# igormq/aes-lac-2018

Measured on AMD Instinct MI355X. Metric: train frames/sec, DeepSpeech2 5xBiGRU-800, higher is better.
Workload: dtype f32

## Files before the change

### aes-lac-2018_amd/csrc/bn.hip

```cpp
#include "ds2_common.h"

namespace {

constexpr int NPART = 64;

template <int MODE>
__global__ __launch_bounds__(256) void bn2d_reduce_kernel(const float* __restrict__ x, const float* __restrict__ dy,
                                                          const float* __restrict__ mean_invstd,
                                                          const float* __restrict__ gamma,
                                                          const float* __restrict__ beta, int B, int C, int inner,
                                                          double* __restrict__ part) {
    const int c = blockIdx.y, p = blockIdx.x, tid = threadIdx.x;
    const int chunks = (inner + 1023) / 1024;
    const int items = B * chunks;
    float mu = 0.f, is = 0.f, ga = 0.f, be = 0.f;
    if (MODE == 1) {
        mu = mean_invstd[c];
        is = mean_invstd[C + c];
        ga = gamma[c];
        be = beta[c];
    }
    float s0 = 0.f, s1 = 0.f;
    for (int it = p; it < items; it += NPART) {
        const int b = it / chunks, ch = it % chunks;
        const size_t base = ((size_t)b * C + c) * inner;
        const int i0 = ch * 1024;
#pragma unroll
        for (int u = 0; u < 4; ++u) {
            const int i = i0 + u * 256 + tid;
            if (i < inner) {
                const float v = x[base + i];
                if (MODE == 0) {
                    s0 += v;
                    s1 += v * v;
                } else {
                    const float xh = (v - mu) * is;
                    const float y = ga * xh + be;
                    const float g = (y > 0.f && y < 20.f) ? dy[base + i] : 0.f;
                    s0 += g;
                    s1 += g * xh;
                }
            }
        }
    }
    double d0 = wave_sum_d((double)s0), d1 = wave_sum_d((double)s1);
    __shared__ double sm[4][2];
    if ((tid & 63) == 0) {
        sm[tid >> 6][0] = d0;
        sm[tid >> 6][1] = d1;
    }
    __syncthreads();
    if (tid == 0) {
        part[((size_t)c * NPART + p) * 2 + 0] = sm[0][0] + sm[1][0] + sm[2][0] + sm[3][0];
        part[((size_t)c * NPART + p) * 2 + 1] = sm[0][1] + sm[1][1] + sm[2][1] + sm[3][1];
    }
}

template <int MODE>
__global__ __launch_bounds__(256) void bn2d_reduce_vec_kernel(const float* __restrict__ x, const float* __restrict__ dy,
                                                              const float* __restrict__ mean_invstd,
                                                              const float* __restrict__ gamma,
                                                              const float* __restrict__ beta, int B, int C, int inner,
                                                              double* __restrict__ part) {
    const int c = blockIdx.y, p = blockIdx.x, tid = threadIdx.x;
    const int chunks = (inner + 1023) / 1024;
    const int items = B * chunks;
    float mu = 0.f, is = 0.f, ga = 0.f, be = 0.f;
    if (MODE == 1) {
        mu = mean_invstd[c];
        is = mean_invstd[C + c];
        ga = gamma[c];
        be = beta[c];
    }
    float s0 = 0.f, s1 = 0.f;
    auto take = [&](float v, float g) {
        if (MODE == 0) {
            s0 += v;
            s1 += v * v;
        } else {
            const float xh = (v - mu) * is;
            const float y = ga * xh + be;
            const float gm = (y > 0.f && y < 20.f) ? g : 0.f;
            s0 += gm;
            s1 += gm * xh;
        }
    };
    for (int it = p; it < items; it += NPART) {
        const int b = it / chunks, ch = it % chunks;
        const size_t base = ((size_t)b * C + c) * inner;
        const int h = min((int)((4 - (base & 3)) & 3), inner);
        const int nq = (inner - h) >> 2;
        const int q = ch * 256 + tid;
        if (q < nq) {
            const f32x4 v = *reinterpret_cast<const f32x4*>(x + base + h + 4 * (size_t)q);
            f32x4 g = {0.f, 0.f, 0.f, 0.f};
            if (MODE == 1) g = *reinterpret_cast<const f32x4*>(dy + base + h + 4 * (size_t)q);
#pragma unroll
            for (int e = 0; e < 4; ++e) take(v[e], g[e]);
        }
        if (ch == 0) {
            const int tail0 = h + 4 * nq, e = tid < 4 ? tid : tail0 + tid - 4;
            if ((tid < h) || (tid >= 4 && tid < 8 && e < inner)) take(x[base + e], MODE == 1 ? dy[base + e] : 0.f);
        }
    }
    double d0 = wave_sum_d((double)s0), d1 = wave_sum_d((double)s1);
    __shared__ double sm[4][2];
    if ((tid & 63) == 0) {
        sm[tid >> 6][0] = d0;
        sm[tid >> 6][1] = d1;
    }
    __syncthreads();
    if (tid == 0) {
        part[((size_t)c * NPART + p) * 2 + 0] = sm[0][0] + sm[1][0] + sm[2][0] + sm[3][0];
        part[((size_t)c * NPART + p) * 2 + 1] = sm[0][1] + sm[1][1] + sm[2][1] + sm[3][1];
    }
}

template <int MODE>
__global__ __launch_bounds__(256) void bn1d_reduce_kernel(const float* __restrict__ xa, const float* __restrict__ xb,
                                                          const float* __restrict__ dy,
                                                          const float* __restrict__ mean_invstd, int rows, int F,
                                                          double* __restrict__ part) {
    const int p = blockIdx.x, tid = threadIdx.x;
    const int col = blockIdx.y * 64 + (tid & 63), ry = tid >> 6;
    float mu = 0.f, is = 0.f;
    if (MODE == 1 && col < F) {
        mu = mean_invstd[col];
        is = mean_invstd[F + col];
    }
    float s0 = 0.f, s1 = 0.f;
    if (col < F) {
        for (int r = p * 4 + ry; r < rows; r += NPART * 4) {
            const size_t o = (size_t)r * F + col;
            float v = xa[o];
            if (xb) v += xb[o];
            if (MODE == 0) {
                s0 += v;
                s1 += v * v;
            } else {
                const float g = dy[o];
                s0 += g;
                s1 += g * (v - mu) * is;
            }
        }
    }
    __shared__ float sm[4][64][2];
    sm[ry][tid & 63][0] = s0;
    sm[ry][tid & 63][1] = s1;
    __syncthreads();
    if (ry == 0 && col < F) {
        const int l = tid & 63;
        const double d0 = (double)sm[0][l][0] + (double)sm[1][l][0] + (double)sm[2][l][0] + (double)sm[3][l][0];
        const double d1 = (double)sm[0][l][1] + (double)sm[1][l][1] + (double)sm[2][l][1] + (double)sm[3][l][1];
        part[((size_t)col * NPART + p) * 2 + 0] = d0;
        part[((size_t)col * NPART + p) * 2 + 1] = d1;
    }
}

__global__ __launch_bounds__(64) void bn_finalize_stats_kernel(const double* __restrict__ part, int C, double count,
                                                               float eps, float momentum, int use_running,
                                                               float* __restrict__ running_mean,
                                                               float* __restrict__ running_var,
                                                               float* __restrict__ mean_invstd) {
    const int c = blockIdx.x, lane = threadIdx.x;
    if (use_running) {
        if (lane == 0) {
            mean_invstd[c] = running_mean[c];
            mean_invstd[C + c] = (float)(1.0 / sqrt((double)running_var[c] + (double)eps));
        }
        return;
    }
    double s0 = part[((size_t)c * NPART + lane) * 2 + 0];
    double s1 = part[((size_t)c * NPART + lane) * 2 + 1];
    s0 = wave_sum_d(s0);
    s1 = wave_sum_d(s1);
    if (lane == 0) {
        const double mean = s0 / count;
        double var = s1 / count - mean * mean;
        if (var < 0.0) var = 0.0;
        mean_invstd[c] = (float)mean;
        mean_invstd[C + c] = (float)(1.0 / sqrt(var + (double)eps));
        if (running_mean) {
            const double unb = count > 1.0 ? var * count / (count - 1.0) : var;
            running_mean[c] = (float)((1.0 - momentum) * running_mean[c] + momentum * mean);
            running_var[c] = (float)((1.0 - momentum) * running_var[c] + momentum * unb);
        }
    }
}

__global__ __launch_bounds__(64) void bn_finalize_bwd_kernel(const double* __restrict__ part, int C, double count,
                                                             float* __restrict__ dgamma, float* __restrict__ dbeta,
                                                             float* __restrict__ coef) {
    const int c = blockIdx.x, lane = threadIdx.x;
    double s0 = part[((size_t)c * NPART + lane) * 2 + 0];
    double s1 = part[((size_t)c * NPART + lane) * 2 + 1];
    s0 = wave_sum_d(s0);
    s1 = wave_sum_d(s1);
    if (lane == 0) {
        dbeta[c] = (float)s0;
        dgamma[c] = (float)s1;
        coef[c] = (float)(s0 / count);
        coef[C + c] = (float)(s1 / count);
    }
}

__global__ __launch_bounds__(256) void bn2d_apply_kernel(const float* __restrict__ x,
                                                         const float* __restrict__ mean_invstd,
                                                         const float* __restrict__ gamma,
                                                         const float* __restrict__ beta, int C, int inner,
                                                         float* __restrict__ y) {
    const int bc = blockIdx.y, c = bc % C;
    const float sc = gamma[c] * mean_invstd[C + c];
    const float sh = beta[c] - mean_invstd[c] * sc;
    const size_t base = (size_t)bc * inner;
    for (int i = blockIdx.x * 256 + threadIdx.x; i < inner; i += gridDim.x * 256) {
        const float v = x[base + i] * sc + sh;
        y[base + i] = fminf(fmaxf(v, 0.f), 20.f);
    }
}

__global__ __launch_bounds__(256) void bn2d_apply_tbf_kernel(const float* __restrict__ x,
                                                             const float* __restrict__ mean_invstd,
                                                             const float* __restrict__ gamma,
                                                             const float* __restrict__ beta, int B, int C, int D,
                                                             int T, float* __restrict__ y) {
    __shared__ float tile[32][33];
    const int b = blockIdx.z;
    const int CD = C * D;
    const int t0 = blockIdx.x * 32, f0 = blockIdx.y * 32;
    const int tx = threadIdx.x & 31, ty = threadIdx.x >> 5;
#pragma unroll
    for (int i = 0; i < 32; i += 8) {
        const int f = f0 + ty + i, t = t0 + tx;
        if (f < CD && t < T) {
            const int c = f / D;
            const float sc = gamma[c] * mean_invstd[C + c];
            const float sh = beta[c] - mean_invstd[c] * sc;
            const float v = x[((size_t)b * CD + f) * T + t] * sc + sh;
            tile[ty + i][tx] = fminf(fmaxf(v, 0.f), 20.f);
        }
    }
    __syncthreads();
#pragma unroll
    for (int i = 0; i < 32; i += 8) {
        const int t = t0 + ty + i, f = f0 + tx;
        if (f < CD && t < T) y[((size_t)t * B + b) * CD + f] = tile[tx][ty + i];
    }
}

__global__ __launch_bounds__(256) void bn2d_bwd_apply_kernel(const float* __restrict__ x, const float* __restrict__ dy,
                                                             const float* __restrict__ mean_invstd,
                                                             const float* __restrict__ gamma,
                                                             const float* __restrict__ beta,
                                                             const float* __restrict__ coef, int C, int inner,
                                                             float* __restrict__ dx) {
    const int bc = blockIdx.y, c = bc % C;
    const float mu = mean_invstd[c], is = mean_invstd[C + c], ga = gamma[c], be = beta[c];
    const float mg = coef[c], mgx = coef[C + c];
    const size_t base = (size_t)bc * inner;
    for (int i = blockIdx.x * 256 + threadIdx.x; i < inner; i += gridDim.x * 256) {
        const float xh = (x[base + i] - mu) * is;
        const float yv = ga * xh + be;
        const float g = (yv > 0.f && yv < 20.f) ? dy[base + i] : 0.f;
        dx[base + i] = ga * is * (g - mg - xh * mgx);
    }
}

template <typename F>
__device__ __forceinline__ void bn2d_row_vec(size_t base, int inner, F&& f4, int bx, int nbx, int tid) {
    const int h = min((int)((4 - (base & 3)) & 3), inner);
    const int nq = (inner - h) >> 2;
    for (int q = bx * 256 + tid; q < nq; q += nbx * 256) f4(base + h + 4 * (size_t)q, 4);
    if (bx == 0) {
        const int tail0 = h + 4 * nq, e = tid < 4 ? tid : tail0 + tid - 4;
        if ((tid < h) || (tid >= 4 && tid < 8 && e < inner)) f4(base + e, 1);
    }
}

__global__ __launch_bounds__(256) void bn2d_bwd_apply_vec_kernel(const float* __restrict__ x, const float* __restrict__ dy,
                                                                 const float* __restrict__ mean_invstd,
                                                                 const float* __restrict__ gamma,
                                                                 const float* __restrict__ beta,
                                                                 const float* __restrict__ coef, int C, int inner,
                                                                 float* __restrict__ dx) {
    const int bc = blockIdx.y, c = bc % C;
    const float mu = mean_invstd[c], is = mean_invstd[C + c], ga = gamma[c], be = beta[c];
    const float mg = coef[c], mgx = coef[C + c];
    auto one = [&](float xv, float g) {
        const float xh = (xv - mu) * is;
        const float yv = ga * xh + be;
        const float gm = (yv > 0.f && yv < 20.f) ? g : 0.f;
        return ga * is * (gm - mg - xh * mgx);
    };
    bn2d_row_vec((size_t)bc * inner, inner, [&](size_t o, int n) {
        if (n == 4) {
            const f32x4 xv = *reinterpret_cast<const f32x4*>(x + o), g = *reinterpret_cast<const f32x4*>(dy + o);
            f32x4 r;
#pragma unroll
            for (int e = 0; e < 4; ++e) r[e] = one(xv[e], g[e]);
            *reinterpret_cast<f32x4*>(dx + o) = r;
        } else {
            dx[o] = one(x[o], dy[o]);
        }
    }, blockIdx.x, gridDim.x, threadIdx.x);
}

__global__ __launch_bounds__(256) void bn2d_apply_vec_kernel(const float* __restrict__ x,
                                                             const float* __restrict__ mean_invstd,
                                                             const float* __restrict__ gamma,
                                                             const float* __restrict__ beta, int C, int inner,
                                                             float* __restrict__ y) {
    const int bc = blockIdx.y, c = bc % C;
    const float sc = gamma[c] * mean_invstd[C + c];
    const float sh = beta[c] - mean_invstd[c] * sc;
    bn2d_row_vec((size_t)bc * inner, inner, [&](size_t o, int n) {
        if (n == 4) {
            const f32x4 xv = *reinterpret_cast<const f32x4*>(x + o);
            f32x4 r;
#pragma unroll
            for (int e = 0; e < 4; ++e) r[e] = fminf(fmaxf(xv[e] * sc + sh, 0.f), 20.f);
            *reinterpret_cast<f32x4*>(y + o) = r;
        } else {
            y[o] = fminf(fmaxf(x[o] * sc + sh, 0.f), 20.f);
        }
    }, blockIdx.x, gridDim.x, threadIdx.x);
}

__global__ __launch_bounds__(256) void bn1d_apply_kernel(const float* __restrict__ xa, const float* __restrict__ xb,
                                                         const float* __restrict__ mean_invstd,
                                                         const float* __restrict__ gamma,
                                                         const float* __restrict__ beta, size_t n, int F,
                                                         float* __restrict__ y) {
    const size_t stride = (size_t)gridDim.x * 256;
    for (size_t i = (size_t)blockIdx.x * 256 + threadIdx.x; i < n; i += stride) {
        const int col = (int)(i % F);
        float v = xa[i];
        if (xb) v += xb[i];
        const float sc = gamma[col] * mean_invstd[F + col];
        y[i] = (v - mean_invstd[col]) * sc + beta[col];
    }
}

__global__ __launch_bounds__(256) void bn1d_bwd_apply_kernel(const float* __restrict__ xa, const float* __restrict__ xb,
                                                             const float* __restrict__ dy,
                                                             const float* __restrict__ mean_invstd,
                                                             const float* __restrict__ gamma,
                                                             const float* __restrict__ coef, size_t n, int F,
                                                             float* __restrict__ dx) {
    const size_t stride = (size_t)gridDim.x * 256;
    for (size_t i = (size_t)blockIdx.x * 256 + threadIdx.x; i < n; i += stride) {
        const int col = (int)(i % F);
        float v = xa[i];
        if (xb) v += xb[i];
        const float is = mean_invstd[F + col];
        const float xh = (v - mean_invstd[col]) * is;
        dx[i] = gamma[col] * is * (dy[i] - coef[col] - xh * coef[F + col]);
    }
}

template <int MODE>
__global__ __launch_bounds__(256) void bn1d_reduce_vec_kernel(const f32x4* __restrict__ xa, const f32x4* __restrict__ xb,
                                                              const f32x4* __restrict__ dy,
                                                              const float* __restrict__ mean_invstd, int rows, int F,
                                                              double* __restrict__ part) {
    const int p = blockIdx.x, tid = threadIdx.x;
    const int F4 = F >> 2;
    const int cq = blockIdx.y * 64 + (tid & 63), ry = tid >> 6;
    f32x4 mu = {0.f, 0.f, 0.f, 0.f}, is = mu;
    if (MODE == 1 && cq < F4) {
        mu = *reinterpret_cast<const f32x4*>(mean_invstd + 4 * cq);
        is = *reinterpret_cast<const f32x4*>(mean_invstd + F + 4 * cq);
    }
    f32x4 s0 = {0.f, 0.f, 0.f, 0.f}, s1 = s0;
    if (cq < F4) {
        for (int r = p * 4 + ry; r < rows; r += NPART * 4) {
            const size_t o = (size_t)r * F4 + cq;
            f32x4 v = xa[o];
            if (xb) v += xb[o];
            if (MODE == 0) {
                s0 += v;
                s1 += v * v;
            } else {
                const f32x4 g = dy[o];
                s0 += g;
                s1 += g * (v - mu) * is;
            }
        }
    }
    __shared__ f32x4 sm[4][64][2];
    sm[ry][tid & 63][0] = s0;
    sm[ry][tid & 63][1] = s1;
    __syncthreads();
    if (ry == 0 && cq < F4) {
        const int l = tid & 63;
#pragma unroll
        for (int e = 0; e < 4; ++e) {
            const double d0 = (double)sm[0][l][0][e] + (double)sm[1][l][0][e] + (double)sm[2][l][0][e] + (double)sm[3][l][0][e];
            const double d1 = (double)sm[0][l][1][e] + (double)sm[1][l][1][e] + (double)sm[2][l][1][e] + (double)sm[3][l][1][e];
            part[((size_t)(4 * cq + e) * NPART + p) * 2 + 0] = d0;
            part[((size_t)(4 * cq + e) * NPART + p) * 2 + 1] = d1;
        }
    }
}

__global__ __launch_bounds__(256) void bn1d_apply_vec_kernel(const f32x4* __restrict__ xa, const f32x4* __restrict__ xb,
                                                             const float* __restrict__ mean_invstd,
                                                             const float* __restrict__ gamma,
                                                             const float* __restrict__ beta, size_t n4, int F4,
                                                             f32x4* __restrict__ y) {
    const size_t stride = (size_t)gridDim.x * 256;
    for (size_t i = (size_t)blockIdx.x * 256 + threadIdx.x; i < n4; i += stride) {
        const int c = 4 * (int)(i % F4);
        f32x4 v = xa[i];
        if (xb) v += xb[i];
        const f32x4 sc = *reinterpret_cast<const f32x4*>(gamma + c) * *reinterpret_cast<const f32x4*>(mean_invstd + 4 * F4 + c);
        y[i] = (v - *reinterpret_cast<const f32x4*>(mean_invstd + c)) * sc + *reinterpret_cast<const f32x4*>(beta + c);
    }
}

__global__ __launch_bounds__(256) void bn1d_bwd_apply_vec_kernel(const f32x4* __restrict__ xa, const f32x4* __restrict__ xb,
                                                                 const f32x4* __restrict__ dy,
                                                                 const float* __restrict__ mean_invstd,
                                                                 const float* __restrict__ gamma,
                                                                 const float* __restrict__ coef, size_t n4, int F4,
                                                                 f32x4* __restrict__ dx) {
    const size_t stride = (size_t)gridDim.x * 256;
    const int F = 4 * F4;
    for (size_t i = (size_t)blockIdx.x * 256 + threadIdx.x; i < n4; i += stride) {
        const int c = 4 * (int)(i % F4);
        f32x4 v = xa[i];
        if (xb) v += xb[i];
        const f32x4 is = *reinterpret_cast<const f32x4*>(mean_invstd + F + c);
        const f32x4 xh = (v - *reinterpret_cast<const f32x4*>(mean_invstd + c)) * is;
        dx[i] = *reinterpret_cast<const f32x4*>(gamma + c) * is *
                (dy[i] - *reinterpret_cast<const f32x4*>(coef + c) - xh * *reinterpret_cast<const f32x4*>(coef + F + c));
    }
}

inline bool aligned16(const void* p) { return ((uintptr_t)p & 15) == 0; }
inline bool vec4_ok(int F, const void* a, const void* b, const void* c, const void* d) {
    return (F & 3) == 0 && ((((uintptr_t)a) | ((uintptr_t)b) | ((uintptr_t)c) | ((uintptr_t)d)) & 15) == 0;
}

inline int ew_blocks(size_t n) {
    size_t b = (n + 255) / 256;
    if (b > 4096) b = 4096;
    if (b < 1) b = 1;
    return (int)b;
}

}

extern "C" size_t ds2_bn_ws_bytes(int C) { return (size_t)C * NPART * 2 * sizeof(double) + (size_t)C * 2 * sizeof(float); }

extern "C" int ds2_bn2d_stats(const float* x, int B, int C, int inner, float eps, float momentum, int use_running,
                              float* running_mean, float* running_var, float* mean_invstd, void* ws, void* stream) {
    DS2_CHECK_ARG(x && mean_invstd && ws && B > 0 && C > 0 && inner > 0);
    DS2_CHECK_ARG(!use_running || (running_mean && running_var));
    hipStream_t st = (hipStream_t)stream;
    double* part = (double*)ws;
    if (!use_running) {
        if (aligned16(x))
            hipLaunchKernelGGL((bn2d_reduce_vec_kernel<0>), dim3(NPART, C), dim3(256), 0, st, x, nullptr, nullptr, nullptr,
                               nullptr, B, C, inner, part);
        else
            hipLaunchKernelGGL((bn2d_reduce_kernel<0>), dim3(NPART, C), dim3(256), 0, st, x, nullptr, nullptr, nullptr,
                               nullptr, B, C, inner, part);
    }
    hipLaunchKernelGGL(bn_finalize_stats_kernel, dim3(C), dim3(64), 0, st, part, C, (double)B * inner, eps, momentum,
                       use_running, running_mean, running_var, mean_invstd);
    DS2_CHECK_LAUNCH();
    return DS2_OK;
}

extern "C" int ds2_bn2d_apply_htanh(const float* x, const float* mean_invstd, const float* gamma, const float* beta,
                                    int B, int C, int D, int T, int layout_tbf, float* y, void* stream) {
    DS2_CHECK_ARG(x && mean_invstd && gamma && beta && y && B > 0 && C > 0 && D > 0 && T > 0);
    hipStream_t st = (hipStream_t)stream;
    if (layout_tbf) {
        DS2_CHECK_ARG(B <= 65535);
        dim3 grid(ds2_cdiv(T, 32), ds2_cdiv(C * D, 32), B);
        hipLaunchKernelGGL(bn2d_apply_tbf_kernel, grid, dim3(256), 0, st, x, mean_invstd, gamma, beta, B, C, D, T, y);
    } else {
        const int inner = D * T;
        if (aligned16(x) && aligned16(y)) {
            dim3 grid(min(ds2_cdiv(inner, 1024), 64), B * C);
            hipLaunchKernelGGL(bn2d_apply_vec_kernel, grid, dim3(256), 0, st, x, mean_invstd, gamma, beta, C, inner, y);
        } else {
            dim3 grid(min(ds2_cdiv(inner, 256), 64), B * C);
            hipLaunchKernelGGL(bn2d_apply_kernel, grid, dim3(256), 0, st, x, mean_invstd, gamma, beta, C, inner, y);
        }
    }
    DS2_CHECK_LAUNCH();
    return DS2_OK;
}

extern "C" int ds2_bn2d_htanh_bwd(const float* x, const float* dy, const float* mean_invstd, const float* gamma,
                                  const float* beta, int B, int C, int D, int T, float* dx, float* dgamma,
                                  float* dbeta, void* ws, void* stream) {
    DS2_CHECK_ARG(x && dy && mean_invstd && gamma && beta && dx && dgamma && dbeta && ws);
    DS2_CHECK_ARG(B > 0 && C > 0 && D > 0 && T > 0);
    hipStream_t st = (hipStream_t)stream;
    const int inner = D * T;
    double* part = (double*)ws;
    float* coef = (float*)(part + (size_t)C * NPART * 2);
    const bool vec = aligned16(x) && aligned16(dy) && aligned16(dx);
    if (vec)
        hipLaunchKernelGGL((bn2d_reduce_vec_kernel<1>), dim3(NPART, C), dim3(256), 0, st, x, dy, mean_invstd, gamma, beta,
                           B, C, inner, part);
    else
        hipLaunchKernelGGL((bn2d_reduce_kernel<1>), dim3(NPART, C), dim3(256), 0, st, x, dy, mean_invstd, gamma, beta, B,
                           C, inner, part);
    hipLaunchKernelGGL(bn_finalize_bwd_kernel, dim3(C), dim3(64), 0, st, part, C, (double)B * inner, dgamma, dbeta,
                       coef);
    if (vec) {
        dim3 grid(min(ds2_cdiv(inner, 1024), 64), B * C);
        hipLaunchKernelGGL(bn2d_bwd_apply_vec_kernel, grid, dim3(256), 0, st, x, dy, mean_invstd, gamma, beta, coef, C,
                           inner, dx);
    } else {
        dim3 grid(min(ds2_cdiv(inner, 256), 64), B * C);
        hipLaunchKernelGGL(bn2d_bwd_apply_kernel, grid, dim3(256), 0, st, x, dy, mean_invstd, gamma, beta, coef, C, inner,
                           dx);
    }
    DS2_CHECK_LAUNCH();
    return DS2_OK;
}

extern "C" int ds2_bn1d_stats(const float* xa, const float* xb, int rows, int F, float eps, float momentum,
                              int use_running, float* running_mean, float* running_var, float* mean_invstd, void* ws,
                              void* stream) {
    DS2_CHECK_ARG(xa && mean_invstd && ws && rows > 0 && F > 0);
    DS2_CHECK_ARG(!use_running || (running_mean && running_var));
    hipStream_t st = (hipStream_t)stream;
    double* part = (double*)ws;
    if (!use_running) {
        if (vec4_ok(F, xa, xb, nullptr, nullptr))
            hipLaunchKernelGGL((bn1d_reduce_vec_kernel<0>), dim3(NPART, ds2_cdiv(F / 4, 64)), dim3(256), 0, st,
                               (const f32x4*)xa, (const f32x4*)xb, nullptr, nullptr, rows, F, part);
        else
            hipLaunchKernelGGL((bn1d_reduce_kernel<0>), dim3(NPART, ds2_cdiv(F, 64)), dim3(256), 0, st, xa, xb, nullptr,
                               nullptr, rows, F, part);
    }
    hipLaunchKernelGGL(bn_finalize_stats_kernel, dim3(F), dim3(64), 0, st, part, F, (double)rows, eps, momentum,
                       use_running, running_mean, running_var, mean_invstd);
    DS2_CHECK_LAUNCH();
    return DS2_OK;
}

extern "C" int ds2_bn1d_apply(const float* xa, const float* xb, const float* mean_invstd, const float* gamma,
                              const float* beta, int rows, int F, float* y, void* stream) {
    DS2_CHECK_ARG(xa && mean_invstd && gamma && beta && y && rows > 0 && F > 0);
    const size_t n = (size_t)rows * F;
    if (vec4_ok(F, xa, xb, y, gamma) && vec4_ok(F, beta, mean_invstd, nullptr, nullptr))
        hipLaunchKernelGGL(bn1d_apply_vec_kernel, dim3(ew_blocks(n / 4)), dim3(256), 0, (hipStream_t)stream,
                           (const f32x4*)xa, (const f32x4*)xb, mean_invstd, gamma, beta, n / 4, F / 4, (f32x4*)y);
    else
        hipLaunchKernelGGL(bn1d_apply_kernel, dim3(ew_blocks(n)), dim3(256), 0, (hipStream_t)stream, xa, xb,
                           mean_invstd, gamma, beta, n, F, y);
    DS2_CHECK_LAUNCH();
    return DS2_OK;
}

extern "C" int ds2_bn1d_bwd(const float* xa, const float* xb, const float* dy, const float* mean_invstd,
                            const float* gamma, int rows, int F, float* dx, float* dgamma, float* dbeta, void* ws,
                            void* stream) {
    DS2_CHECK_ARG(xa && dy && mean_invstd && gamma && dx && dgamma && dbeta && ws && rows > 0 && F > 0);
    hipStream_t st = (hipStream_t)stream;
    double* part = (double*)ws;
    float* coef = (float*)(part + (size_t)F * NPART * 2);
    const bool vec = vec4_ok(F, xa, xb, dy, dx) && vec4_ok(F, gamma, mean_invstd, nullptr, nullptr);
    if (vec)
        hipLaunchKernelGGL((bn1d_reduce_vec_kernel<1>), dim3(NPART, ds2_cdiv(F / 4, 64)), dim3(256), 0, st,
                           (const f32x4*)xa, (const f32x4*)xb, (const f32x4*)dy, mean_invstd, rows, F, part);
    else
        hipLaunchKernelGGL((bn1d_reduce_kernel<1>), dim3(NPART, ds2_cdiv(F, 64)), dim3(256), 0, st, xa, xb, dy,
                           mean_invstd, rows, F, part);
    hipLaunchKernelGGL(bn_finalize_bwd_kernel, dim3(F), dim3(64), 0, st, part, F, (double)rows, dgamma, dbeta, coef);
    const size_t n = (size_t)rows * F;
    if (vec)
        hipLaunchKernelGGL(bn1d_bwd_apply_vec_kernel, dim3(ew_blocks(n / 4)), dim3(256), 0, st, (const f32x4*)xa,
                           (const f32x4*)xb, (const f32x4*)dy, mean_invstd, gamma, coef, n / 4, F / 4, (f32x4*)dx);
    else
        hipLaunchKernelGGL(bn1d_bwd_apply_kernel, dim3(ew_blocks(n)), dim3(256), 0, st, xa, xb, dy, mean_invstd, gamma,
                           coef, n, F, dx);
    DS2_CHECK_LAUNCH();
    return DS2_OK;
}
```

### aes-lac-2018_amd/ds2hip/ops.py

```python
import os

import torch

from . import lib

F_BINS = 161
BN_EPS = 1e-5
BN_MOMENTUM = 0.1


def _empty(shape, like, dtype=torch.float32):
    return torch.empty(shape, dtype=dtype, device=like.device)


def _bytes_ws(nbytes, like):
    return torch.empty((int(nbytes) + 15) // 16 * 2, dtype=torch.float64, device=like.device)


def conv_out_frames(t_in):
    t1 = (t_in + 20 - 11) // 2 + 1
    return t1, t1 - 10


def spectrogram(wav, wav_offsets, t_max, normalize=True, eps=1e-9):
# ... 121 lines not shown
            ev.record()
            self.ring[host_tensor.dtype][i] = (buf, ev, False)
        return out

    def stage(self, host_tensor):
        n = host_tensor.numel()
        with self.lock:
            i, buf = self._slot(host_tensor.dtype, n, busy=True)
            view = buf[:n]
            view.copy_(host_tensor.reshape(-1))
        return i, view

    def staged_done(self, dtype, i):
        ev = torch.cuda.Event()
        ev.record()
        with self.lock:
            self.ring[dtype][i] = (self.ring[dtype][i][0], ev, False)

    def download(self, dev_tensor):
        n = dev_tensor.numel()
        with self.lock:
            i, buf = self._slot(dev_tensor.dtype, n)
            buf[:n].copy_(dev_tensor.reshape(-1), non_blocking=True)
            ev = torch.cuda.Event()
            ev.record()
            self.ring[dev_tensor.dtype][i] = (buf, ev, False)
        return buf[:n], ev


_pinned = _PinnedRing()
_staged = _PinnedRing()


def upload_small(host_tensor, device):
    return _pinned.upload(host_tensor, device)


def download_small(dev_tensor):
    return _pinned.download(dev_tensor)


def spin_wait(event):
    import time
    while not event.query():
        time.sleep(0)


def low_priority_stream(device):
    import ctypes
    with torch.cuda.device(device):
        out = ctypes.c_void_p()
        rc = lib.load().ds2_stream_create(1, ctypes.byref(out))
        if rc != 0:
            raise RuntimeError('ds2_stream_create failed (%d): %s' % (rc, lib.load().ds2_last_error().decode()))
        return torch.cuda.ExternalStream(out.value, device=device)

def gemm(a, b, trans_a=False, trans_b=False, out=None, beta=0.0, m=None, n=None, k=None, lda=None, ldb=None,
         ldc=None, split_k=1):
    if m is None:
        m = a.shape[1] if trans_a else a.shape[0]
    if k is None:
        k = a.shape[0] if trans_a else a.shape[1]
    if n is None:
        n = b.shape[0] if trans_b else b.shape[1]
    if lda is None:
        lda = a.shape[-1]
    if ldb is None:
        ldb = b.shape[-1]
    if out is None:
        out = _empty((m, n), a)
    if ldc is None:
        ldc = out.shape[-1]
    lib.call('ds2_gemm_f32', int(trans_a), int(trans_b), m, n, k, a, lda, b, ldb, out, ldc, float(beta), split_k)
    return out


def gemm_split_mode(mode=-1):
    return int(lib.load().ds2_gemm_split_mode(int(mode)))


def gemm_raw(trans_a, trans_b, m, n, k, a_ptr, lda, b_ptr, ldb, c_ptr, ldc, beta=0.0, split_k=1):
    lib.call('ds2_gemm_f32', int(trans_a), int(trans_b), m, n, k, a_ptr, lda, b_ptr, ldb, c_ptr, ldc, float(beta),
             split_k)


def gemm_tn_group(problems, n, k, accumulate=False):
    import ctypes
    cnt = len(problems)
    assert 1 <= cnt <= 4
    vp, ip = ctypes.c_void_p * cnt, ctypes.c_int * cnt
    a, lda, m, b, ldb, c, ldc = zip(*problems)
    args = (vp(*a), ip(*lda), ip(*m), vp(*b), ip(*ldb), vp(*c), ip(*ldc))
    fn = lib.load().ds2_gemm_f32_tn_group
    rc = fn(cnt, *[ctypes.cast(x, ctypes.c_void_p) for x in args], int(n), int(k), int(bool(accumulate)),
            lib.stream_ptr())
    if rc != 0:
        raise lib.Ds2Error(rc, 'ds2_gemm_f32_tn_group failed (%d): %s' % (rc, lib.load().ds2_last_error().decode()))


def transpose2d(x, rows, cols, out=None):
    if out is None:
        out = _empty((cols, rows), x)
    lib.call('ds2_transpose2d', x, rows, cols, out)
    return out


def transpose2d_group(tensors, batch, rows, cols, out):
    import ctypes
    cnt = len(tensors)
    assert 1 <= cnt <= 8 and all(t.is_cuda and t.is_contiguous() and t.numel() == batch * rows * cols for t in tensors)
    assert out.is_cuda and out.is_contiguous() and out.numel() == cnt * batch * rows * cols
    ptrs = (ctypes.c_void_p * cnt)(*[t.data_ptr() for t in tensors])
    rc = lib.load().ds2_transpose2d_group(cnt, ctypes.cast(ptrs, ctypes.c_void_p), int(batch), int(rows), int(cols),
                                          out.data_ptr(), lib.stream_ptr())
    if rc != 0:
        raise lib.Ds2Error(rc, 'ds2_transpose2d_group failed (%d): %s' % (rc, lib.load().ds2_last_error().decode()))
    return out


def add2(a, b):
    out = torch.empty_like(a)
    lib.call('ds2_add2', a, b, a.numel(), out)
    return out


def transpose_btf(x):
    bsz, t, f = x.shape
    out = _empty((bsz, f, t), x)
    lib.call('ds2_transpose_btf_to_bft', x, bsz, t, f, out)
    return out


def conv_fwd(which, inp, weight, bias, t_in):
    bsz = inp.shape[0]
    t1, t2 = conv_out_frames(t_in) if which == 1 else (None, t_in - 10)
    out = _empty((bsz, 32, 61, t1), inp) if which == 1 else _empty((bsz, 32, 21, t2), inp)
    ws = _empty((lib.query('ds2_conv_wt_ws_floats', which),), inp)
    lib.call('ds2_conv_fwd', which, inp, weight, bias, bsz, t_in, out, ws)
    return out


def conv2_dgrad(d_out, weight, t1):
    bsz = d_out.shape[0]
    d_in = _empty((bsz, 32, 61, t1), d_out)
    ws = _empty((lib.query('ds2_conv2_dgrad_ws_floats', bsz, t1),), d_out)
    lib.call('ds2_conv2_dgrad', d_out, weight, bsz, t1, d_in, ws, ws.numel())
    return d_in


def conv_wgrad(which, inp, d_out, t_in, d_weight, d_bias):
    lib.call('ds2_conv_wgrad', which, inp, d_out, inp.shape[0], t_in, d_weight, d_bias)


def _bn_ws(c, like):
    return _bytes_ws(lib.query('ds2_bn_ws_bytes', c), like)


def bn2d_stats(x, running_mean, running_var, training):
    bsz, c = x.shape[0], x.shape[1]
    inner = x.numel() // (bsz * c)
    mi = _empty((2 * c,), x)
    lib.call('ds2_bn2d_stats', x, bsz, c, inner, BN_EPS, BN_MOMENTUM, int(not training), running_mean, running_var, mi,
             _bn_ws(c, x))
    return mi


def bn2d_apply_htanh(x, mi, gamma, beta, layout_tbf):
    bsz, c, d, t = x.shape
    y = _empty((t, bsz, c * d), x) if layout_tbf else torch.empty_like(x)
    lib.call('ds2_bn2d_apply_htanh', x, mi, gamma, beta, bsz, c, d, t, int(layout_tbf), y)
    return y


def bn2d_htanh_bwd(x, dy, mi, gamma, beta, dgamma, dbeta):
    bsz, c, d, t = x.shape
    dx = torch.empty_like(x)
    lib.call('ds2_bn2d_htanh_bwd', x, dy, mi, gamma, beta, bsz, c, d, t, dx, dgamma, dbeta, _bn_ws(c, x))
    return dx


def bn1d_stats(xa, xb, rows, feat, running_mean, running_var, training):
    mi = _empty((2 * feat,), xa)
    lib.call('ds2_bn1d_stats', xa, xb, rows, feat, BN_EPS, BN_MOMENTUM, int(not training), running_mean, running_var,
             mi, _bn_ws(feat, xa))
    return mi


def bn1d_apply(xa, xb, mi, gamma, beta, rows, feat):
    y = _empty((rows, feat), xa)
    lib.call('ds2_bn1d_apply', xa, xb, mi, gamma, beta, rows, feat, y)
    return y


def bn1d_bwd(xa, xb, dy, mi, gamma, rows, feat, dgamma, dbeta):
    dx = _empty((rows, feat), xa)
    lib.call('ds2_bn1d_bwd', xa, xb, dy, mi, gamma, rows, feat, dx, dgamma, dbeta, _bn_ws(feat, xa))
    return dx


def _host_ints(vals):
    import ctypes
    return ctypes.cast((ctypes.c_int * len(vals))(*[int(v) for v in vals]), ctypes.c_void_p)


def _host_ptrs(tensors):
    import ctypes
    ptrs = []
    for t in tensors:
        if t is not None:
            assert t.is_cuda and t.is_contiguous()
        ptrs.append(None if t is None else t.data_ptr())
    return ctypes.cast((ctypes.c_void_p * len(ptrs))(*ptrs), ctypes.c_void_p)


def bn1d_seg_stats(xa, xb, t, bsz, feat, bounds, running_means, running_vars, training):
    g = len(bounds) - 1
    mi = _empty((g, 2 * feat), xa)
    lib.call('ds2_bn1d_seg_stats', xa, xb, t, bsz, feat, g, _host_ints(bounds), BN_EPS, BN_MOMENTUM, int(not training),
             _host_ptrs(running_means), _host_ptrs(running_vars), mi, _bytes_ws(g * lib.query('ds2_bn_ws_bytes', feat), xa))
    return mi


def bn1d_seg_apply(xa, xb, mi, t, bsz, feat, bounds, gammas, betas):
    y = _empty((t * bsz, feat), xa)
    lib.call('ds2_bn1d_seg_apply', xa, xb, mi, t, bsz, feat, len(bounds) - 1, _host_ints(bounds), _host_ptrs(gammas),
             _host_ptrs(betas), y)
    return y


def bn1d_seg_bwd(xa, xb, dxf, mi, t, bsz, feat, bounds, gammas, dgammas, dbetas):
    g = len(bounds) - 1
    dy = _empty((t * bsz, feat), xa)
    lib.call('ds2_bn1d_seg_bwd', xa, xb, dxf, mi, t, bsz, feat, g, _host_ints(bounds), _host_ptrs(gammas), dy,
             _host_ptrs(dgammas), _host_ptrs(dbetas), _bytes_ws(g * lib.query('ds2_bn_ws_bytes', feat), xa))
    return dy


GRU_MODE = os.environ.get('DS2_GRU_MODE', 'auto')
_sync_ws = {}
fallback_count = 0
_persistent_off = {}


def _dev_key(dev):
    return (dev.type, dev.index if dev.index is not None else torch.cuda.current_device())


def _gru_sync_ws(dev, bsz, hid):
    key = _dev_key(dev)
    n = (lib.query('ds2_gru_sync_ws_bytes', bsz, hid) + 3) // 4
    if key not in _sync_ws or _sync_ws[key].numel() < n:
        old = _sync_ws.get(key)
        if old is not None:
            word = lib.query('ds2_gru_sync_error_offset') // 4
            if int(old[word].item()) != 0:
                raise_async_error()
            _err_ptr_tables.clear()
        _sync_ws[key] = torch.zeros(n, dtype=torch.int32, device=dev)
    return _sync_ws[key]


def _use_persistent(dev, bsz, hid):
    if GRU_MODE == 'step':
        return False
    if _dev_key(dev) in _persistent_off:
        if GRU_MODE == 'persistent':
            raise RuntimeError('persistent GRU kernels are disabled on %s: %s' % (dev, _persistent_off[_dev_key(dev)]))
        return False
    ok = bool(lib.query('ds2_gru_persistent_supported', bsz, hid))
    if GRU_MODE == 'persistent' and not ok:
        raise RuntimeError('persistent GRU kernel does not support B=%d H=%d on this device' % (bsz, hid))
    return ok


def _disable_persistent(dev, reason):
    import logging
    global fallback_count
    fallback_count += 1
    if os.environ.get('DS2_GRU_STRICT', '0') == '1':
        raise RuntimeError('ds2hip: the persistent GRU kernels would fall back to the launch-per-step kernels on %s (%s) '
                           'and DS2_GRU_STRICT=1 forbids it' % (dev, reason))
    _persistent_off[_dev_key(dev)] = reason
    logging.getLogger('aes-lac-2018').warning('ds2hip: persistent GRU kernels disabled on %s (%s); using the '
                                              'launch-per-step kernels', dev, reason)


def async_error_words():
    word = lib.query('ds2_gru_sync_error_offset') // 4
    return [ws[word:word + 1] for ws in _sync_ws.values()]


def raise_async_error():
    for key, ws in _sync_ws.items():
        word = lib.query('ds2_gru_sync_error_offset') // 4
        bad = int(ws[word].item()) != 0
        ws.zero_()
        if bad:
            _disable_persistent(ws.device, 'a hand-off spin timed out (were all workgroups resident?)')
    raise RuntimeError('ds2hip: persistent GRU kernel timed out waiting for a workgroup hand-off; the results of this '
                       'step are invalid')


def check_async_errors():
    for w in async_error_words():
        if int(w.item()) != 0:
            raise_async_error()


_dh_supported = {}


def gru_bwd_dh_wanted(dev, bsz, hid):
    if not _use_persistent(dev, bsz, hid):
        return False
    key = (bsz, hid)
    if key not in _dh_supported:
        _dh_supported[key] = bool(lib.query('ds2_gru_bwd_dh_supported', bsz, hid))
    if not _dh_supported[key]:
        return False
    e = os.environ.get('DS2_GRU_BWD_DH')
    if e in ('0', '1'):
        return e == '1'
    return bsz >= 9


def gru_bidir_fwd(gates, w_hh, t, bsz, hid, want_coef=False):
    ghn = _empty((t, bsz, 2, hid), gates)
    hout = _empty((2, t, bsz, hid), gates)
    coef = _empty((t, bsz, 2, 3 * hid), gates) if want_coef and gru_bwd_dh_wanted(gates.device, bsz, hid) else None
    if _use_persistent(gates.device, bsz, hid):
        try:
            lib.call('ds2_gru_bidir_fwd_persistent_ex', gates, ghn, hout, w_hh, coef, _gru_sync_ws(gates.device, bsz, hid), t,
                     bsz, hid)
            return (ghn, hout, coef) if want_coef else (ghn, hout)
        except lib.Ds2Error as e:
            if e.code != lib.ERR_UNSUPPORTED or GRU_MODE == 'persistent':
                raise
            _disable_persistent(gates.device, str(e))
    lib.call('ds2_gru_bidir_fwd', gates, ghn, hout, w_hh, t, bsz, hid)
    return (ghn, hout, None) if want_coef else (ghn, hout)


def gru_bwd_coef(gates, ghn, hout, t, bsz, hid):
    coef = _empty((t, bsz, 2, 3 * hid), gates)
    lib.call('ds2_gru_bwd_coef', gates, ghn, hout, coef, t, bsz, hid)
    return coef


def gru_bidir_bwd(gates, ghn, hout, d_out, w_hh_t, t, bsz, hid, spare_cus=-1, coef=None):
# ... 144 lines not shown
```

Baseline: 565,000.

## Fuse BN finalize into reduce kernels via last-block atomic counter

Removes the separate BN finalize kernels. Each reduce kernel stores its partial sums with relaxed atomics, and the last block for each channel, found through an atomic counter, does the final sum and writes the stats or gradient coefficients. The partial layout changes to [p][k][C] to suit the in-kernel sum, and workspaces are cached and zero-initialised per device, stream and channel count so the counters start at zero. This saves one kernel launch per BN call. In exchange it adds atomic and ordering risk and shares cached workspaces between calls with the same channel count.

```diff
diff --git a/aes-lac-2018_amd/csrc/bn.hip b/aes-lac-2018_amd/csrc/bn.hip
--- a/aes-lac-2018_amd/csrc/bn.hip
+++ b/aes-lac-2018_amd/csrc/bn.hip
@@ -3,13 +3,100 @@
 namespace {
 
 constexpr int NPART = 64;
+
+struct BnFinal {
+    unsigned int* counter;
+    double count;
+    float eps, momentum;
+    float* running_mean;
+    float* running_var;
+    float* mi_out;
+    float* dgamma;
+    float* dbeta;
+    float* coef;
+};
+
+__device__ __forceinline__ size_t part_at(int p, int k, int C, int c) { return ((size_t)p * 2 + k) * C + c; }
+
+__device__ __forceinline__ void part_store(double* part, size_t i, double v) {
+    __hip_atomic_store(part + i, v, __ATOMIC_RELAXED, __HIP_MEMORY_SCOPE_AGENT);
+}
+__device__ __forceinline__ double part_load(const double* part, size_t i) {
+    return __hip_atomic_load(part + i, __ATOMIC_RELAXED, __HIP_MEMORY_SCOPE_AGENT);
+}
+
+__device__ __forceinline__ bool bn_last_block(unsigned int* counter, unsigned int total) {
+    __shared__ unsigned int last;
+    if (threadIdx.x < 64) {
+        __builtin_amdgcn_s_waitcnt(0x0F70);
+        asm volatile("" ::: "memory");
+        if (threadIdx.x == 0) {
+            last = atomicAdd(counter, 1u) == total - 1 ? 1u : 0u;
+            if (last) atomicExch(counter, 0u);
+        }
+    }
+    __syncthreads();
+    return last != 0u;
+}
+
+__device__ __forceinline__ double bn_tree_sum(const double* part, int C, int c, int k) {
+    double v[NPART];
+#pragma unroll
+    for (int p = 0; p < NPART; ++p) v[p] = part_load(part, part_at(p, k, C, c));
+#pragma unroll
+    for (int o = NPART / 2; o > 0; o >>= 1)
+#pragma unroll
+        for (int i = 0; i < o; ++i) v[i] += v[i + o];
+    return v[0];
+}
+
+template <int MODE>
+__device__ __forceinline__ void bn_finish(double s0, double s1, int c, int C, const BnFinal& f) {
+    if (MODE == 0) {
+        const double mean = s0 / f.count;
+        double var = s1 / f.count - mean * mean;
+        if (var < 0.0) var = 0.0;
+        f.mi_out[c] = (float)mean;
+        f.mi_out[C + c] = (float)(1.0 / sqrt(var + (double)f.eps));
+        if (f.running_mean) {
+            const double unb = f.count > 1.0 ? var * f.count / (f.count - 1.0) : var;
+            f.running_mean[c] = (float)((1.0 - f.momentum) * f.running_mean[c] + f.momentum * mean);
+            f.running_var[c] = (float)((1.0 - f.momentum) * f.running_var[c] + f.momentum * unb);
+        }
+    } else {
+        f.dbeta[c] = (float)s0;
+        f.dgamma[c] = (float)s1;
+        f.coef[c] = (float)(s0 / f.count);
+        f.coef[C + c] = (float)(s1 / f.count);
+    }
+}
+
+template <int MODE>
+__device__ __forceinline__ void bn2d_finalize(const double* part, int C, int c, const BnFinal& f) {
+    if (!bn_last_block(f.counter + c, NPART)) return;
+    const int lane = threadIdx.x;
+    if (lane >= 64) return;
+    const double s0 = wave_sum_d(part_load(part, part_at(lane, 0, C, c)));
+    const double s1 = wave_sum_d(part_load(part, part_at(lane, 1, C, c)));
+    if (lane == 0) bn_finish<MODE>(s0, s1, c, C, f);
+}
+
+template <int MODE>
+__device__ __forceinline__ void bn1d_finalize(const double* part, int F, int ncols, const BnFinal& f) {
+    if (!bn_last_block(f.counter + blockIdx.y, NPART)) return;
+    const int col = blockIdx.y * ncols + threadIdx.x;
+    if ((int)threadIdx.x >= ncols || col >= F) return;
+    const double s0 = bn_tree_sum(part, F, col, 0);
+    const double s1 = bn_tree_sum(part, F, col, 1);
+    bn_finish<MODE>(s0, s1, col, F, f);
+}
 
 template <int MODE>
 __global__ __launch_bounds__(256) void bn2d_reduce_kernel(const float* __restrict__ x, const float* __restrict__ dy,
                                                           const float* __restrict__ mean_invstd,
                                                           const float* __restrict__ gamma,
                                                           const float* __restrict__ beta, int B, int C, int inner,
-                                                          double* __restrict__ part) {
+                                                          double* part, BnFinal fin) {
     const int c = blockIdx.y, p = blockIdx.x, tid = threadIdx.x;
     const int chunks = (inner + 1023) / 1024;
     const int items = B * chunks;
@@ -51,9 +138,10 @@
     }
     __syncthreads();
     if (tid == 0) {
-        part[((size_t)c * NPART + p) * 2 + 0] = sm[0][0] + sm[1][0] + sm[2][0] + sm[3][0];
-        part[((size_t)c * NPART + p) * 2 + 1] = sm[0][1] + sm[1][1] + sm[2][1] + sm[3][1];
-    }
+        part_store(part, part_at(p, 0, C, c), sm[0][0] + sm[1][0] + sm[2][0] + sm[3][0]);
+        part_store(part, part_at(p, 1, C, c), sm[0][1] + sm[1][1] + sm[2][1] + sm[3][1]);
+    }
+    bn2d_finalize<MODE>(part, C, c, fin);
 }
 
 template <int MODE>
@@ -61,7 +149,7 @@
                                                               const float* __restrict__ mean_invstd,
                                                               const float* __restrict__ gamma,
                                                               const float* __restrict__ beta, int B, int C, int inner,
-                                                              double* __restrict__ part) {
+                                                              double* part, BnFinal fin) {
     const int c = blockIdx.y, p = blockIdx.x, tid = threadIdx.x;
     const int chunks = (inner + 1023) / 1024;
     const int items = B * chunks;
@@ -111,16 +199,17 @@
     }
     __syncthreads();
     if (tid == 0) {
-        part[((size_t)c * NPART + p) * 2 + 0] = sm[0][0] + sm[1][0] + sm[2][0] + sm[3][0];
-        part[((size_t)c * NPART + p) * 2 + 1] = sm[0][1] + sm[1][1] + sm[2][1] + sm[3][1];
-    }
+        part_store(part, part_at(p, 0, C, c), sm[0][0] + sm[1][0] + sm[2][0] + sm[3][0]);
+        part_store(part, part_at(p, 1, C, c), sm[0][1] + sm[1][1] + sm[2][1] + sm[3][1]);
+    }
+    bn2d_finalize<MODE>(part, C, c, fin);
 }
 
 template <int MODE>
 __global__ __launch_bounds__(256) void bn1d_reduce_kernel(const float* __restrict__ xa, const float* __restrict__ xb,
                                                           const float* __restrict__ dy,
                                                           const float* __restrict__ mean_invstd, int rows, int F,
-                                                          double* __restrict__ part) {
+                                                          double* part, BnFinal fin) {
     const int p = blockIdx.x, tid = threadIdx.x;
     const int col = blockIdx.y * 64 + (tid & 63), ry = tid >> 6;
     float mu = 0.f, is = 0.f;
@@ -152,55 +241,19 @@
         const int l = tid & 63;
         const double d0 = (double)sm[0][l][0] + (double)sm[1][l][0] + (double)sm[2][l][0] + (double)sm[3][l][0];
         const double d1 = (double)sm[0][l][1] + (double)sm[1][l][1] + (double)sm[2][l][1] + (double)sm[3][l][1];
-        part[((size_t)col * NPART + p) * 2 + 0] = d0;
-        part[((size_t)col * NPART + p) * 2 + 1] = d1;
-    }
-}
-
-__global__ __launch_bounds__(64) void bn_finalize_stats_kernel(const double* __restrict__ part, int C, double count,
-                                                               float eps, float momentum, int use_running,
-                                                               float* __restrict__ running_mean,
-                                                               float* __restrict__ running_var,
-                                                               float* __restrict__ mean_invstd) {
-    const int c = blockIdx.x, lane = threadIdx.x;
-    if (use_running) {
-        if (lane == 0) {
-            mean_invstd[c] = running_mean[c];
-            mean_invstd[C + c] = (float)(1.0 / sqrt((double)running_var[c] + (double)eps));
-        }
-        return;
-    }
-    double s0 = part[((size_t)c * NPART + lane) * 2 + 0];
-    double s1 = part[((size_t)c * NPART + lane) * 2 + 1];
-    s0 = wave_sum_d(s0);
-    s1 = wave_sum_d(s1);
-    if (lane == 0) {
-        const double mean = s0 / count;
-        double var = s1 / count - mean * mean;
-        if (var < 0.0) var = 0.0;
-        mean_invstd[c] = (float)mean;
-        mean_invstd[C + c] = (float)(1.0 / sqrt(var + (double)eps));
-        if (running_mean) {
-            const double unb = count > 1.0 ? var * count / (count - 1.0) : var;
-            running_mean[c] = (float)((1.0 - momentum) * running_mean[c] + momentum * mean);
-            running_var[c] = (float)((1.0 - momentum) * running_var[c] + momentum * unb);
-        }
-    }
-}
-
-__global__ __launch_bounds__(64) void bn_finalize_bwd_kernel(const double* __restrict__ part, int C, double count,
-                                                             float* __restrict__ dgamma, float* __restrict__ dbeta,
-                                                             float* __restrict__ coef) {
-    const int c = blockIdx.x, lane = threadIdx.x;
-    double s0 = part[((size_t)c * NPART + lane) * 2 + 0];
-    double s1 = part[((size_t)c * NPART + lane) * 2 + 1];
-    s0 = wave_sum_d(s0);
-    s1 = wave_sum_d(s1);
-    if (lane == 0) {
-        dbeta[c] = (float)s0;
-        dgamma[c] = (float)s1;
-        coef[c] = (float)(s0 / count);
-        coef[C + c] = (float)(s1 / count);
+        part_store(part, part_at(p, 0, F, col), d0);
+        part_store(part, part_at(p, 1, F, col), d1);
+    }
+    bn1d_finalize<MODE>(part, F, 64, fin);
+}
+
+__global__ __launch_bounds__(256) void bn_running_stats_kernel(int C, float eps, const float* __restrict__ running_mean,
+                                                              const float* __restrict__ running_var,
+                                                              float* __restrict__ mean_invstd) {
+    const int c = blockIdx.x * 256 + threadIdx.x;
+    if (c < C) {
+        mean_invstd[c] = running_mean[c];
+        mean_invstd[C + c] = (float)(1.0 / sqrt((double)running_var[c] + (double)eps));
     }
 }
 
@@ -362,7 +415,7 @@
 __global__ __launch_bounds__(256) void bn1d_reduce_vec_kernel(const f32x4* __restrict__ xa, const f32x4* __restrict__ xb,
                                                               const f32x4* __restrict__ dy,
                                                               const float* __restrict__ mean_invstd, int rows, int F,
-                                                              double* __restrict__ part) {
+                                                              double* part, BnFinal fin) {
     const int p = blockIdx.x, tid = threadIdx.x;
     const int F4 = F >> 2;
     const int cq = blockIdx.y * 64 + (tid & 63), ry = tid >> 6;
@@ -397,10 +450,11 @@
         for (int e = 0; e < 4; ++e) {
             const double d0 = (double)sm[0][l][0][e] + (double)sm[1][l][0][e] + (double)sm[2][l][0][e] + (double)sm[3][l][0][e];
             const double d1 = (double)sm[0][l][1][e] + (double)sm[1][l][1][e] + (double)sm[2][l][1][e] + (double)sm[3][l][1][e];
-            part[((size_t)(4 * cq + e) * NPART + p) * 2 + 0] = d0;
-            part[((size_t)(4 * cq + e) * NPART + p) * 2 + 1] = d1;
-        }
-    }
+            part_store(part, part_at(p, 0, F, 4 * cq + e), d0);
+            part_store(part, part_at(p, 1, F, 4 * cq + e), d1);
+        }
+    }
+    bn1d_finalize<MODE>(part, F, 256, fin);
 }
 
 __global__ __launch_bounds__(256) void bn1d_apply_vec_kernel(const f32x4* __restrict__ xa, const f32x4* __restrict__ xb,
@@ -451,7 +505,39 @@
 
 }
 
-extern "C" size_t ds2_bn_ws_bytes(int C) { return (size_t)C * NPART * 2 * sizeof(double) + (size_t)C * 2 * sizeof(float); }
+extern "C" size_t ds2_bn_ws_bytes(int C) {
+    return (size_t)C * NPART * 2 * sizeof(double) + (size_t)C * 2 * sizeof(float) + (size_t)C * sizeof(unsigned int);
+}
+
+namespace {
+
+inline float* ws_coef(void* ws, int C) { return (float*)((double*)ws + (size_t)C * NPART * 2); }
+inline unsigned int* ws_counter(void* ws, int C) { return (unsigned int*)(ws_coef(ws, C) + 2 * (size_t)C); }
+
+inline BnFinal final_stats(void* ws, int C, double count, float eps, float momentum, float* running_mean,
+                           float* running_var, float* mean_invstd) {
+    BnFinal f = {};
+    f.counter = ws_counter(ws, C);
+    f.count = count;
+    f.eps = eps;
+    f.momentum = momentum;
+    f.running_mean = running_mean;
+    f.running_var = running_var;
+    f.mi_out = mean_invstd;
+    return f;
+}
+
+inline BnFinal final_bwd(void* ws, int C, double count, float* dgamma, float* dbeta) {
+    BnFinal f = {};
+    f.counter = ws_counter(ws, C);
+    f.count = count;
+    f.dgamma = dgamma;
+    f.dbeta = dbeta;
+    f.coef = ws_coef(ws, C);
+    return f;
+}
+
+}
 
 extern "C" int ds2_bn2d_stats(const float* x, int B, int C, int inner, float eps, float momentum, int use_running,
                               float* running_mean, float* running_var, float* mean_invstd, void* ws, void* stream) {
@@ -459,16 +545,19 @@
     DS2_CHECK_ARG(!use_running || (running_mean && running_var));
     hipStream_t st = (hipStream_t)stream;
     double* part = (double*)ws;
-    if (!use_running) {
+    if (use_running) {
+        hipLaunchKernelGGL(bn_running_stats_kernel, dim3(ds2_cdiv(C, 256)), dim3(256), 0, st, C, eps, running_mean,
+                           running_var, mean_invstd);
+    } else {
+        DS2_CHECK_ARG(C <= 65535);
+        const BnFinal fin = final_stats(ws, C, (double)B * inner, eps, momentum, running_mean, running_var, mean_invstd);
         if (aligned16(x))
             hipLaunchKernelGGL((bn2d_reduce_vec_kernel<0>), dim3(NPART, C), dim3(256), 0, st, x, nullptr, nullptr, nullptr,
-                               nullptr, B, C, inner, part);
+                               nullptr, B, C, inner, part, fin);
         else
             hipLaunchKernelGGL((bn2d_reduce_kernel<0>), dim3(NPART, C), dim3(256), 0, st, x, nullptr, nullptr, nullptr,
-                               nullptr, B, C, inner, part);
-    }
-    hipLaunchKernelGGL(bn_finalize_stats_kernel, dim3(C), dim3(64), 0, st, part, C, (double)B * inner, eps, momentum,
-                       use_running, running_mean, running_var, mean_invstd);
+                               nullptr, B, C, inner, part, fin);
+    }
     DS2_CHECK_LAUNCH();
     return DS2_OK;
 }
@@ -503,16 +592,15 @@
     hipStream_t st = (hipStream_t)stream;
     const int inner = D * T;
     double* part = (double*)ws;
-    float* coef = (float*)(part + (size_t)C * NPART * 2);
+    float* coef = ws_coef(ws, C);
+    const BnFinal fin = final_bwd(ws, C, (double)B * inner, dgamma, dbeta);
     const bool vec = aligned16(x) && aligned16(dy) && aligned16(dx);
     if (vec)
         hipLaunchKernelGGL((bn2d_reduce_vec_kernel<1>), dim3(NPART, C), dim3(256), 0, st, x, dy, mean_invstd, gamma, beta,
-                           B, C, inner, part);
+                           B, C, inner, part, fin);
     else
         hipLaunchKernelGGL((bn2d_reduce_kernel<1>), dim3(NPART, C), dim3(256), 0, st, x, dy, mean_invstd, gamma, beta, B,
-                           C, inner, part);
-    hipLaunchKernelGGL(bn_finalize_bwd_kernel, dim3(C), dim3(64), 0, st, part, C, (double)B * inner, dgamma, dbeta,
-                       coef);
+                           C, inner, part, fin);
     if (vec) {
         dim3 grid(min(ds2_cdiv(inner, 1024), 64), B * C);
         hipLaunchKernelGGL(bn2d_bwd_apply_vec_kernel, grid, dim3(256), 0, st, x, dy, mean_invstd, gamma, beta, coef, C,
@@ -533,16 +621,18 @@
     DS2_CHECK_ARG(!use_running || (running_mean && running_var));
     hipStream_t st = (hipStream_t)stream;
     double* part = (double*)ws;
-    if (!use_running) {
+    if (use_running) {
+        hipLaunchKernelGGL(bn_running_stats_kernel, dim3(ds2_cdiv(F, 256)), dim3(256), 0, st, F, eps, running_mean,
+                           running_var, mean_invstd);
+    } else {
+        const BnFinal fin = final_stats(ws, F, (double)rows, eps, momentum, running_mean, running_var, mean_invstd);
         if (vec4_ok(F, xa, xb, nullptr, nullptr))
             hipLaunchKernelGGL((bn1d_reduce_vec_kernel<0>), dim3(NPART, ds2_cdiv(F / 4, 64)), dim3(256), 0, st,
-                               (const f32x4*)xa, (const f32x4*)xb, nullptr, nullptr, rows, F, part);
+                               (const f32x4*)xa, (const f32x4*)xb, nullptr, nullptr, rows, F, part, fin);
         else
             hipLaunchKernelGGL((bn1d_reduce_kernel<0>), dim3(NPART, ds2_cdiv(F, 64)), dim3(256), 0, st, xa, xb, nullptr,
-                               nullptr, rows, F, part);
-    }
-    hipLaunchKernelGGL(bn_finalize_stats_kernel, dim3(F), dim3(64), 0, st, part, F, (double)rows, eps, momentum,
-                       use_running, running_mean, running_var, mean_invstd);
+                               nullptr, rows, F, part, fin);
+    }
     DS2_CHECK_LAUNCH();
     return DS2_OK;
 }
@@ -567,15 +657,15 @@
     DS2_CHECK_ARG(xa && dy && mean_invstd && gamma && dx && dgamma && dbeta && ws && rows > 0 && F > 0);
     hipStream_t st = (hipStream_t)stream;
     double* part = (double*)ws;
-    float* coef = (float*)(part + (size_t)F * NPART * 2);
+    float* coef = ws_coef(ws, F);
+    const BnFinal fin = final_bwd(ws, F, (double)rows, dgamma, dbeta);
     const bool vec = vec4_ok(F, xa, xb, dy, dx) && vec4_ok(F, gamma, mean_invstd, nullptr, nullptr);
     if (vec)
         hipLaunchKernelGGL((bn1d_reduce_vec_kernel<1>), dim3(NPART, ds2_cdiv(F / 4, 64)), dim3(256), 0, st,
-                           (const f32x4*)xa, (const f32x4*)xb, (const f32x4*)dy, mean_invstd, rows, F, part);
+                           (const f32x4*)xa, (const f32x4*)xb, (const f32x4*)dy, mean_invstd, rows, F, part, fin);
     else
         hipLaunchKernelGGL((bn1d_reduce_kernel<1>), dim3(NPART, ds2_cdiv(F, 64)), dim3(256), 0, st, xa, xb, dy,
-                           mean_invstd, rows, F, part);
-    hipLaunchKernelGGL(bn_finalize_bwd_kernel, dim3(F), dim3(64), 0, st, part, F, (double)rows, dgamma, dbeta, coef);
+                           mean_invstd, rows, F, part, fin);
     const size_t n = (size_t)rows * F;
     if (vec)
         hipLaunchKernelGGL(bn1d_bwd_apply_vec_kernel, dim3(ew_blocks(n / 4)), dim3(256), 0, st, (const f32x4*)xa,
diff --git a/aes-lac-2018_amd/ds2hip/ops.py b/aes-lac-2018_amd/ds2hip/ops.py
--- a/aes-lac-2018_amd/ds2hip/ops.py
+++ b/aes-lac-2018_amd/ds2hip/ops.py
@@ -297,16 +297,29 @@
     lib.call('ds2_conv_wgrad', which, inp, d_out, inp.shape[0], t_in, d_weight, d_bias)
 
 
-def _bn_ws(c, like):
-    return _bytes_ws(lib.query('ds2_bn_ws_bytes', c), like)
-
-
-def bn2d_stats(x, running_mean, running_var, training):
+_bn_ws_cache = {}
+
+
+def bn_workspace(c, like):
+    return torch.zeros((int(lib.query('ds2_bn_ws_bytes', c)) + 15) // 16 * 2, dtype=torch.float64, device=like.device)
+
+
+def _bn_ws(c, like, ws=None):
+    if ws is not None:
+        return ws
+    key = (_dev_key(like.device), lib.stream_ptr(), c)
+    ws = _bn_ws_cache.get(key)
+    if ws is None:
+        ws = _bn_ws_cache[key] = bn_workspace(c, like)
+    return ws
+
+
+def bn2d_stats(x, running_mean, running_var, training, ws=None):
     bsz, c = x.shape[0], x.shape[1]
     inner = x.numel() // (bsz * c)
     mi = _empty((2 * c,), x)
     lib.call('ds2_bn2d_stats', x, bsz, c, inner, BN_EPS, BN_MOMENTUM, int(not training), running_mean, running_var, mi,
-             _bn_ws(c, x))
+             _bn_ws(c, x, ws))
     return mi
 
 
@@ -317,17 +330,17 @@
     return y
 
 
-def bn2d_htanh_bwd(x, dy, mi, gamma, beta, dgamma, dbeta):
+def bn2d_htanh_bwd(x, dy, mi, gamma, beta, dgamma, dbeta, ws=None):
     bsz, c, d, t = x.shape
     dx = torch.empty_like(x)
-    lib.call('ds2_bn2d_htanh_bwd', x, dy, mi, gamma, beta, bsz, c, d, t, dx, dgamma, dbeta, _bn_ws(c, x))
+    lib.call('ds2_bn2d_htanh_bwd', x, dy, mi, gamma, beta, bsz, c, d, t, dx, dgamma, dbeta, _bn_ws(c, x, ws))
     return dx
 
 
-def bn1d_stats(xa, xb, rows, feat, running_mean, running_var, training):
+def bn1d_stats(xa, xb, rows, feat, running_mean, running_var, training, ws=None):
     mi = _empty((2 * feat,), xa)
     lib.call('ds2_bn1d_stats', xa, xb, rows, feat, BN_EPS, BN_MOMENTUM, int(not training), running_mean, running_var,
-             mi, _bn_ws(feat, xa))
+             mi, _bn_ws(feat, xa, ws))
     return mi
 
 
@@ -337,9 +350,9 @@
     return y
 
 
-def bn1d_bwd(xa, xb, dy, mi, gamma, rows, feat, dgamma, dbeta):
+def bn1d_bwd(xa, xb, dy, mi, gamma, rows, feat, dgamma, dbeta, ws=None):
     dx = _empty((rows, feat), xa)
-    lib.call('ds2_bn1d_bwd', xa, xb, dy, mi, gamma, rows, feat, dx, dgamma, dbeta, _bn_ws(feat, xa))
+    lib.call('ds2_bn1d_bwd', xa, xb, dy, mi, gamma, rows, feat, dx, dgamma, dbeta, _bn_ws(feat, xa, ws))
     return dx
 
 
```

After: 551,700. 0.976x the previous value.
